# databendlabs/databend

Measured on AMD Instinct MI355X. Metric: rows/s TPC-H Q1 hash-agg, higher is better.
Workload: dtype i64/i128 decimal

## Files before the change

databend_amd/csrc/dev_common.h:

```cpp
#pragma once
#ifndef __HIPCC_RTC__
#include <hip/hip_runtime.h>
#include <stdint.h>
#endif

#ifndef __HIPCC_RTC__
#include "../../include/dbhip.h"
#else
#include "dbhip.h"
#endif

typedef __int128 i128;
typedef unsigned __int128 u128;

#define DBHIP_WAVE 64

#define DBHIP_NULL_HASH_VAL 0xd1cefa08eb382d69ULL

__host__ __device__ __forceinline__ uint64_t agg_hash_u64(uint64_t x) {
  x ^= x >> 32;
  x *= 0xd6e8feb86659fd93ULL;
  x ^= x >> 32;
  x *= 0xd6e8feb86659fd93ULL;
  x ^= x >> 32;
  return x;
}

__host__ __device__ __forceinline__ uint64_t agg_hash_bytes(const uint8_t* p, uint32_t len) {
  const uint64_t M = 0xc6a4a7935bd1e995ULL;
  const uint64_t SEED = 0xe17a1465ULL;
  const int R = 47;
  uint64_t h = SEED ^ ((uint64_t)len * M);
  uint32_t nblocks = len / 8;
  for (uint32_t i = 0; i < nblocks; ++i) {
    uint64_t k = 0;
    for (int b = 0; b < 8; ++b) k |= (uint64_t)p[i * 8 + b] << (8 * b);
    k *= M;
    k ^= k >> R;
    k *= M;
    h ^= k;
    h *= M;
  }
  uint32_t tail = len - nblocks * 8;
  const uint8_t* t = p + nblocks * 8;
  for (uint32_t i = 0; i < tail; ++i) h ^= (uint64_t)t[i] << (8 * (tail - i - 1));
  h ^= h >> R;
  h *= M;
  h ^= h >> R;
  return h;
}

__device__ __forceinline__ uint64_t agg_hash_inline_view(uint32_t len, uint32_t w1, uint32_t w2,
                                                         uint32_t w3) {
  const uint64_t M = 0xc6a4a7935bd1e995ULL;
  const uint64_t SEED = 0xe17a1465ULL;
  const int R = 47;
  uint64_t h = SEED ^ ((uint64_t)len * M);
  uint64_t lo = ((uint64_t)w2 << 32) | w1;
  uint32_t tail_len = len;
  uint64_t tail_src = lo;
  if (len >= 8) {
    uint64_t k = lo;
    k *= M;
    k ^= k >> R;
    k *= M;
    h ^= k;
    h *= M;
    tail_len = len - 8;
    tail_src = w3;
  }
  uint64_t folded = 0;
  for (uint32_t i = 0; i < 7; ++i) {
    if (i < tail_len) folded |= ((tail_src >> (8 * i)) & 0xff) << (8 * (tail_len - i - 1));
  }
  h ^= folded;
  h ^= h >> R;
  h *= M;
  h ^= h >> R;
  return h;
}

__host__ __device__ __forceinline__ uint64_t agg_hash_i256(uint64_t w0, uint64_t w1, uint64_t w2, uint64_t w3) {
  const uint64_t M = 0xc6a4a7935bd1e995ULL;
  const uint64_t SEED = 0xe17a1465ULL;
  const int R = 47;
  uint64_t h = SEED ^ (32ULL * M);
  const uint64_t w[4] = {w0, w1, w2, w3};
#pragma unroll
  for (int i = 0; i < 4; ++i) {
    uint64_t k = w[i];
    k *= M;
    k ^= k >> R;
    k *= M;
    h ^= k;
    h *= M;
  }
  h ^= h >> R;
  h *= M;
  h ^= h >> R;
  return h;
}

__device__ __forceinline__ uint64_t agg_hash_i128(i128 v) {
  const uint64_t M = 0xc6a4a7935bd1e995ULL;
  const uint64_t SEED = 0xe17a1465ULL;
  const int R = 47;
  uint64_t h = SEED ^ (16ULL * M);
  uint64_t w[2] = {(uint64_t)(u128)v, (uint64_t)((u128)v >> 64)};
#pragma unroll
  for (int i = 0; i < 2; ++i) {
    uint64_t k = w[i];
    k *= M;
    k ^= k >> R;
    k *= M;
    h ^= k;
    h *= M;
  }
  h ^= h >> R;
  h *= M;
  h ^= h >> R;
  return h;
}

__host__ __device__ __forceinline__ uint64_t merge_hash(uint64_t a, uint64_t b) {
  return a * DBHIP_NULL_HASH_VAL ^ b;
}

__device__ __forceinline__ bool bit_get(const uint8_t* bm, int64_t i) {
  return (bm[i >> 3] >> (i & 7)) & 1;
}

__device__ __forceinline__ uint64_t wave_sum_u64(uint64_t v) {
#pragma unroll
  for (int off = 32; off >= 1; off >>= 1) v += __shfl_xor(v, off, 64);
  return v;
}

__device__ __forceinline__ u128 wave_sum_u128(u128 v) {
#pragma unroll
  for (int off = 32; off >= 1; off >>= 1) {
    uint64_t lo = __shfl_xor((uint64_t)v, off, 64);
    uint64_t hi = __shfl_xor((uint64_t)(v >> 64), off, 64);
    v += ((u128)hi << 64) | lo;
  }
  return v;
}

__device__ __forceinline__ u128 wave_sum_u192(u128 v, uint64_t* ext) {
  uint64_t e = *ext;
#pragma unroll
  for (int off = 32; off >= 1; off >>= 1) {
    uint64_t lo = __shfl_xor((uint64_t)v, off, 64);
    uint64_t hi = __shfl_xor((uint64_t)(v >> 64), off, 64);
    uint64_t oe = __shfl_xor(e, off, 64);
    u128 o = ((u128)hi << 64) | lo;
    u128 r = v + o;
    e += oe + (r < v ? 1 : 0);
    v = r;
  }
  *ext = e;
  return v;
}

__device__ __forceinline__ int lane_id() { return threadIdx.x & 63; }

struct u256 {
  u128 lo, hi;
};

__host__ __device__ __forceinline__ u256 u256_mul_128(u128 a, u128 b) {
  uint64_t a0 = (uint64_t)a, a1 = (uint64_t)(a >> 64);
  uint64_t b0 = (uint64_t)b, b1 = (uint64_t)(b >> 64);
  u128 p00 = (u128)a0 * b0;
  u128 p01 = (u128)a0 * b1;
  u128 p10 = (u128)a1 * b0;
  u128 p11 = (u128)a1 * b1;
  u128 mid = (p00 >> 64) + (uint64_t)p01 + (uint64_t)p10;
  u256 r;
  r.lo = ((u128)(uint64_t)mid << 64) | (uint64_t)p00;
  r.hi = p11 + (p01 >> 64) + (p10 >> 64) + (mid >> 64);
  return r;
}

__host__ __device__ __forceinline__ u256 u256_add_128(u256 a, u128 b) {
  u256 r;
  r.lo = a.lo + b;
  r.hi = a.hi + (r.lo < a.lo ? 1 : 0);
  return r;
}

__host__ __device__ __forceinline__ bool u256_lt_128(u256 a, u128 b) { return a.hi == 0 && a.lo < b; }

__host__ __device__ __forceinline__ u256 u256_sub_128(u256 a, u128 b) {
  u256 r;
  r.lo = a.lo - b;
  r.hi = a.hi - (a.lo < b ? 1 : 0);
  return r;
}

__host__ __device__ inline uint64_t udiv_2by1(uint64_t u1, uint64_t u0, uint64_t v, uint64_t* rem) {
  const double dv = (double)v;
  const double e = ((double)u1 * 18446744073709551616.0 + (double)u0) / dv;
  uint64_t q = e >= 18446744073709549568.0 ? ~0ULL : (uint64_t)e;
  const u128 n = ((u128)u1 << 64) | u0;
  i128 r = (i128)(n - (u128)q * (u128)v);
  const u128 mag = r < 0 ? (u128)0 - (u128)r : (u128)r;
  const double dm = (double)(uint64_t)(mag >> 64) * 18446744073709551616.0 + (double)(uint64_t)mag;
  const double er = (r < 0 ? -dm : dm) / dv;
  int64_t c = (int64_t)er;
  if ((double)c > er) --c;
  q += (uint64_t)c;
  r -= (i128)c * (i128)(u128)v;
  if (r < 0) { --q; r += (i128)(u128)v; }
  else if (r >= (i128)(u128)v) { ++q; r -= (i128)(u128)v; }
  if (rem) *rem = (uint64_t)r;
  return q;
}

__host__ __device__ inline u128 udiv128_by_64(u128 n, uint64_t d, uint64_t* rem) {
  const uint64_t nh = (uint64_t)(n >> 64), nl = (uint64_t)n;
  uint64_t r = 0;
  const uint64_t qh = nh ? udiv_2by1(0, nh, d, &r) : 0;
  const uint64_t ql = udiv_2by1(r, nl, d, rem);
  return ((u128)qh << 64) | ql;
}

__host__ __device__ inline u256 u256_div_128(u256 a, u128 d, u128* rem) {
  u256 q;
  q.lo = 0;
  q.hi = 0;
  if (a.hi == 0) {
    if ((uint64_t)(d >> 64) == 0) {
      uint64_t r64;
      q.lo = udiv128_by_64(a.lo, (uint64_t)d, &r64);
      if (rem) *rem = r64;
      return q;
    }
    q.lo = a.lo / d;
    if (rem) *rem = a.lo % d;
    return q;
  }
  u128 r = 0;
  for (int i = 255; i >= 0; --i) {
    bool carry = (r >> 127) & 1;
    r <<= 1;
    u128 bit = (i >= 128) ? ((a.hi >> (i - 128)) & 1) : ((a.lo >> i) & 1);
    r |= bit;
    if (carry || r >= d) {
      r -= d;
      if (i >= 128)
        q.hi |= ((u128)1 << (i - 128));
      else
        q.lo |= ((u128)1 << i);
    }
  }
  if (rem) *rem = r;
  return q;
}

static __device__ const uint64_t kDbhipPow10[39][2] = {
  {0x0000000000000001ULL, 0x0000000000000000ULL},
  {0x000000000000000aULL, 0x0000000000000000ULL},
  {0x0000000000000064ULL, 0x0000000000000000ULL},
  {0x00000000000003e8ULL, 0x0000000000000000ULL},
  {0x0000000000002710ULL, 0x0000000000000000ULL},
  {0x00000000000186a0ULL, 0x0000000000000000ULL},
  {0x00000000000f4240ULL, 0x0000000000000000ULL},
  {0x0000000000989680ULL, 0x0000000000000000ULL},
  {0x0000000005f5e100ULL, 0x0000000000000000ULL},
  {0x000000003b9aca00ULL, 0x0000000000000000ULL},
  {0x00000002540be400ULL, 0x0000000000000000ULL},
  {0x000000174876e800ULL, 0x0000000000000000ULL},
  {0x000000e8d4a51000ULL, 0x0000000000000000ULL},
  {0x000009184e72a000ULL, 0x0000000000000000ULL},
  {0x00005af3107a4000ULL, 0x0000000000000000ULL},
  {0x00038d7ea4c68000ULL, 0x0000000000000000ULL},
  {0x002386f26fc10000ULL, 0x0000000000000000ULL},
  {0x016345785d8a0000ULL, 0x0000000000000000ULL},
  {0x0de0b6b3a7640000ULL, 0x0000000000000000ULL},
  {0x8ac7230489e80000ULL, 0x0000000000000000ULL},
  {0x6bc75e2d63100000ULL, 0x0000000000000005ULL},
  {0x35c9adc5dea00000ULL, 0x0000000000000036ULL},
  {0x19e0c9bab2400000ULL, 0x000000000000021eULL},
  {0x02c7e14af6800000ULL, 0x000000000000152dULL},
  {0x1bcecceda1000000ULL, 0x000000000000d3c2ULL},
  {0x161401484a000000ULL, 0x0000000000084595ULL},
  {0xdcc80cd2e4000000ULL, 0x000000000052b7d2ULL},
  {0x9fd0803ce8000000ULL, 0x00000000033b2e3cULL},
  {0x3e25026110000000ULL, 0x00000000204fce5eULL},
  {0x6d7217caa0000000ULL, 0x00000001431e0faeULL},
  {0x4674edea40000000ULL, 0x0000000c9f2c9cd0ULL},
  {0xc0914b2680000000ULL, 0x0000007e37be2022ULL},
  {0x85acef8100000000ULL, 0x000004ee2d6d415bULL},
  {0x38c15b0a00000000ULL, 0x0000314dc6448d93ULL},
  {0x378d8e6400000000ULL, 0x0001ed09bead87c0ULL},
  {0x2b878fe800000000ULL, 0x0013426172c74d82ULL},
  {0xb34b9f1000000000ULL, 0x00c097ce7bc90715ULL},
  {0x00f436a000000000ULL, 0x0785ee10d5da46d9ULL},
  {0x098a224000000000ULL, 0x4b3b4ca85a86c47aULL}};
__host__ __device__ __forceinline__ i128 pow10_i128(int k) {
#if defined(__HIP_DEVICE_COMPILE__)
  k = k < 0 ? 0 : (k > 38 ? 38 : k);
  return (i128)(((u128)kDbhipPow10[k][1] << 64) | kDbhipPow10[k][0]);
#else
  i128 r = 1;
  for (int i = 0; i < k; ++i) r *= 10;
  return r;
#endif
}
```

databend_amd/csrc/dev_decimal.h:

```cpp
#pragma once
#include "dev_common.h"

struct DecOp {
  int op;
  int a_from_scale, a_to_scale, a_to_precision, a_check;
  int b_from_scale, b_to_scale, b_to_precision, b_check;
  int t_is_128;
  int ret_precision, ret_scale;
  int overflow;
  int scale_mul;
  int trivial;
};

__host__ __device__ __forceinline__ i128 wrap_T(i128 v, bool t128) { return t128 ? v : (i128)(int64_t)v; }

__host__ __device__ __forceinline__ i128 max_for_precision(int p) { return pow10_i128(p) - 1; }

__host__ __device__ __forceinline__ bool checked_mul_T(i128 x, i128 f, bool t128, i128* out) {
  if (!t128) {
    i128 r = x * f;
    if (r > (i128)INT64_MAX || r < (i128)INT64_MIN) return false;
    *out = r;
    return true;
  }
  bool neg = (x < 0) != (f < 0);
  u128 ax = x < 0 ? (u128)0 - (u128)x : (u128)x;
  u128 af = f < 0 ? (u128)0 - (u128)f : (u128)f;
  u256 pr = u256_mul_128(ax, af);
  u128 lim = neg ? ((u128)1 << 127) : (((u128)1 << 127) - 1);
  if (pr.hi != 0 || pr.lo > lim) return false;
  *out = neg ? (i128)((u128)0 - pr.lo) : (i128)pr.lo;
  return true;
}

__host__ __device__ __forceinline__ bool convert_operand(i128 x, bool is_decimal, int from_scale, int to_scale,
                                                int to_precision, int check, bool t128, i128* out) {
  if (!is_decimal) {
    if (to_scale == 0) {
      *out = wrap_T(x, t128);
      return true;
    }
    i128 xt = x;
    if (!t128 && (x > (i128)INT64_MAX || x < (i128)INT64_MIN)) return false;
    i128 r;
    if (!checked_mul_T(xt, pow10_i128(to_scale), t128, &r)) return false;
    i128 mx = max_for_precision(to_precision);
    if (r > mx || r < -mx) return false;
    *out = r;
    return true;
  }
  if (!check) {
    *out = wrap_T(x, t128);
    return true;
  }
  i128 r;
  if (!checked_mul_T(wrap_T(x, t128), pow10_i128(to_scale - from_scale), t128, &r)) return false;
  i128 mx = max_for_precision(to_precision);
  if (r > mx || r < -mx) return false;
  *out = r;
  return true;
}

__host__ __device__ __forceinline__ i128 sdiv128(i128 num, i128 d) {
  const bool neg = (num < 0) != (d < 0);
  const u128 un = num < 0 ? (u128)0 - (u128)num : (u128)num;
  const u128 ud = d < 0 ? (u128)0 - (u128)d : (u128)d;
  u128 q;
  if ((uint64_t)(ud >> 64) == 0) q = udiv128_by_64(un, (uint64_t)ud, nullptr);
  else q = un / ud;
  return neg ? (i128)((u128)0 - q) : (i128)q;
}

__device__ bool round_mul_128_overflow(i128 a, i128 b, int shift, i128* out) {
  bool neg = (a < 0) != (b < 0);
  u128 A = a < 0 ? (u128)0 - (u128)a : (u128)a;
  u128 B = b < 0 ? (u128)0 - (u128)b : (u128)b;
  u128 div = (u128)pow10_i128(shift);
  u256 pr = u256_add_128(u256_mul_128(A, B), div / 2);
  u256 q = u256_div_128(pr, div, nullptr);
  u128 lim = neg ? ((u128)1 << 127) : (((u128)1 << 127) - 1);
  if (q.hi != 0 || q.lo > lim) return false;
  *out = neg ? (i128)((u128)0 - q.lo) : (i128)q.lo;
  return true;
}

__device__ i128 round_div_128(i128 a, i128 b, int mul_scale) {
  bool neg = (a < 0) != (b < 0);
  u128 A = a < 0 ? (u128)0 - (u128)a : (u128)a;
  u128 B = b < 0 ? (u128)0 - (u128)b : (u128)b;
  u256 num = u256_add_128(u256_mul_128(A, (u128)pow10_i128(mul_scale)), B / 2);
  u256 q = u256_div_128(num, B, nullptr);
  return neg ? (i128)((u128)0 - q.lo) : (i128)q.lo;
}

__device__ __forceinline__ bool dec_row(const DecOp& p, i128 av, i128 bv, bool a_dec, bool b_dec, bool t128, i128* out) {
  i128 a, b, r = 1;
    bool ok = convert_operand(av, a_dec, p.a_from_scale,
                              p.a_to_scale, p.a_to_precision, p.a_check, t128, &a);
    ok = convert_operand(bv, b_dec, p.b_from_scale,
                         p.b_to_scale, p.b_to_precision, p.b_check, t128, &b) && ok;
    if (ok) {
      switch (p.op) {
        case DBHIP_OP_PLUS:
        case DBHIP_OP_MINUS: {
          i128 t = p.op == DBHIP_OP_PLUS ? (i128)((u128)a + (u128)b) : (i128)((u128)a - (u128)b);
          t = wrap_T(t, t128);
          if (p.overflow) {
            i128 mx = max_for_precision(p.ret_precision);
            if (t < -mx || t > mx) ok = false;
          }
          r = t;
        } break;
        case DBHIP_OP_MULTIPLY: {
          if (p.scale_mul == 0) {
            r = wrap_T((i128)((u128)a * (u128)b), t128);
          } else if (!t128) {
            i128 div = pow10_i128(p.scale_mul);
            if (!p.overflow) {
              int64_t prod = (int64_t)((uint64_t)(int64_t)a * (uint64_t)(int64_t)b);
              int64_t d = (int64_t)div;
              int64_t num = ((a < 0) == (b < 0)) ? (int64_t)((uint64_t)prod + (uint64_t)(d / 2))
                                                 : (int64_t)((uint64_t)prod - (uint64_t)(d / 2));
              r = (i128)(num / d);
            } else {
              i128 num = ((a < 0) == (b < 0)) ? a * b + div / 2 : a * b - div / 2;
              i128 res = sdiv128(num, div);
              i128 mx = max_for_precision(18);
              if (res < -mx || res > mx) ok = false;
              r = res;
            }
          } else {
            if (!p.overflow) {
              i128 div = pow10_i128(p.scale_mul);
              i128 prod = (i128)((u128)a * (u128)b);
              i128 num = ((a < 0) == (b < 0)) ? (i128)((u128)prod + (u128)(div / 2))
                                              : (i128)((u128)prod - (u128)(div / 2));
              r = sdiv128(num, div);
            } else {
              ok = round_mul_128_overflow(a, b, p.scale_mul, &r);
            }
          }
        } break;
        default: {
          if (b == 0) {
            ok = false;
          } else if (!t128) {
            i128 mul = pow10_i128(p.scale_mul);
            i128 am = (i128)((u128)a * (u128)mul);
            i128 num = ((a < 0) == (b < 0)) ? (i128)((u128)am + (u128)(b / 2))
                                            : (i128)((u128)am - (u128)(b / 2));
            r = (i128)(int64_t)sdiv128(num, b);
          } else {
            r = round_div_128(a, b, p.scale_mul);
          }
        } break;
      }
    }
    *out = r;
    return ok;
}


__device__ __forceinline__ bool dec_row_nodiv(const DecOp& p, i128 av, i128 bv, bool a_dec, bool b_dec, bool t128, i128* out) {
  i128 a, b, r = 1;
  bool ok = convert_operand(av, a_dec, p.a_from_scale, p.a_to_scale, p.a_to_precision, p.a_check, t128, &a);
  ok = convert_operand(bv, b_dec, p.b_from_scale, p.b_to_scale, p.b_to_precision, p.b_check, t128, &b) && ok;
  if (ok) {
    if (p.op == DBHIP_OP_MULTIPLY) {
      r = wrap_T((i128)((u128)a * (u128)b), t128);
    } else {
      i128 t = p.op == DBHIP_OP_PLUS ? (i128)((u128)a + (u128)b) : (i128)((u128)a - (u128)b);
      t = wrap_T(t, t128);
      if (p.overflow) {
        const i128 mx = max_for_precision(p.ret_precision);
        if (t < -mx || t > mx) ok = false;
      }
      r = t;
    }
  }
  *out = r;
  return ok;
}
__host__ __device__ inline bool dec_op_needs_division(const DecOp& p) { return p.op == DBHIP_OP_DIVIDE || (p.op == DBHIP_OP_MULTIPLY && p.scale_mul != 0); }

int32_t dbhip_decimal_decode_internal(int op, int a_type, int a_prec, int a_scale, int b_type, int b_prec, int b_scale,
                                      DecOp* out, int* out_type, int* out_precision, int* out_scale);
```

Baseline: 95.18 billion.

## Use precomputed reciprocal division for decimal power-of-ten scaling

Replaces the double-based 128-by-64 division with a Moller-Granlund style reciprocal-multiply 2-by-1 division. Normalized divisors and reciprocals for powers of ten up to 10^19 are precomputed in a device table. Decimal multiply rescaling and the 256-bit overflow path use this table instead of the generic division. Wave-uniform ballot checks skip the high-word division when no lane needs it, at the cost of extra code and a table lookup.

Measured after the change: 95.19 billion (median of 3 runs). Within noise of the previous version (+0.0%).

```diff
diff --git a/databend_amd/csrc/dev_common.h b/databend_amd/csrc/dev_common.h
--- a/databend_amd/csrc/dev_common.h
+++ b/databend_amd/csrc/dev_common.h
@@ -217,25 +217,101 @@
   return q;
 }
 
+struct UdivPre {
+  uint64_t dn, v;
+  uint32_t s;
+};
+
+#if defined(UDIV_WAVE_ANY)
+#elif defined(__HIP_DEVICE_COMPILE__)
+#define UDIV_WAVE_ANY(c) (__builtin_amdgcn_ballot_w64(c) != 0)
+#else
+#define UDIV_WAVE_ANY(c) (c)
+#endif
+
+__host__ __device__ inline UdivPre udiv_pre_make(uint64_t d) {
+  UdivPre p;
+  p.s = (uint32_t)__builtin_clzll(d);
+  p.dn = d << p.s;
+  const uint64_t dn = p.dn;
+  const double x = 18446744073709551616.0 / (double)dn;
+  const double v0 = (x - 1.0) * 18446744073709551616.0 - 16384.0;
+  uint64_t v = (uint64_t)(v0 < 0.0 ? 0.0 : v0);
+  u128 R = ~(u128)0 - (((u128)dn << 64) + (u128)v * (u128)dn);
+  const double dm = (double)(uint32_t)(R >> 64) * 18446744073709551616.0 + (double)(uint64_t)R;
+  uint32_t c = (uint32_t)(dm * x * 5.421010862427522170037e-20);
+  c = c ? c - 1 : 0;
+  v += c;
+  R -= (u128)((uint64_t)c * (dn >> 32)) * 4294967296ULL + (uint64_t)c * (uint64_t)(uint32_t)dn;
+  if (R >= (u128)dn) { ++v; R -= (u128)dn; }
+  if (R >= (u128)dn) { ++v; R -= (u128)dn; }
+  p.v = v;
+  return p;
+}
+
+__host__ __device__ __forceinline__ uint64_t udiv_2by1_pre(uint64_t u1, uint64_t u0, uint64_t dn, uint64_t v, uint64_t* rem) {
+  const u128 q = (u128)v * (u128)u1 + (((u128)u1 << 64) | u0);
+  uint64_t q1 = (uint64_t)(q >> 64) + 1;
+  uint64_t r = u0 - q1 * dn;
+  if (r > (uint64_t)q) { --q1; r += dn; }
+  if (r >= dn) { ++q1; r -= dn; }
+  *rem = r;
+  return q1;
+}
+
+__host__ __device__ inline u128 udiv128_by_64_pre(u128 n, const UdivPre& p, uint64_t* rem) {
+  const uint64_t nh = (uint64_t)(n >> 64), nl = (uint64_t)n;
+  const uint32_t s = p.s;
+  const uint64_t n2 = (nh >> 1) >> (63 - s);
+  const uint64_t n1 = (nh << s) | ((nl >> 1) >> (63 - s));
+  const uint64_t n0 = nl << s;
+  uint64_t qh = 0, r = n1;
+  if (UDIV_WAVE_ANY(n2 != 0 || n1 >= p.dn)) qh = udiv_2by1_pre(n2, n1, p.dn, p.v, &r);
+  const uint64_t ql = udiv_2by1_pre(r, n0, p.dn, p.v, &r);
+  if (rem) *rem = r >> s;
+  return ((u128)qh << 64) | ql;
+}
+
+__host__ __device__ inline void udiv256_by_64_pre(u128 hi, u128 lo, const UdivPre& p, u128* qhi, u128* qlo, uint64_t* rem) {
+  if (!UDIV_WAVE_ANY(hi != 0)) {
+    *qhi = 0;
+    *qlo = udiv128_by_64_pre(lo, p, rem);
+    return;
+  }
+  const uint32_t s = p.s;
+  u128 h = hi, l = lo, qh = 0, ql = 0;
+  uint64_t r = ((uint64_t)(h >> 64) >> 1) >> (63 - s);
+#pragma unroll 1
+  for (int i = 0; i < 4; ++i) {
+    const uint64_t w = ((uint64_t)(h >> 64) << s) | (((uint64_t)h >> 1) >> (63 - s));
+    const uint64_t q = udiv_2by1_pre(r, w, p.dn, p.v, &r);
+    qh = (qh << 64) | (ql >> 64);
+    ql = (ql << 64) | q;
+    h = (h << 64) | (l >> 64);
+    l <<= 64;
+  }
+  *qhi = qh;
+  *qlo = ql;
+  if (rem) *rem = r >> s;
+}
+
 __host__ __device__ inline u128 udiv128_by_64(u128 n, uint64_t d, uint64_t* rem) {
-  const uint64_t nh = (uint64_t)(n >> 64), nl = (uint64_t)n;
-  uint64_t r = 0;
-  const uint64_t qh = nh ? udiv_2by1(0, nh, d, &r) : 0;
-  const uint64_t ql = udiv_2by1(r, nl, d, rem);
-  return ((u128)qh << 64) | ql;
+  const UdivPre p = udiv_pre_make(d);
+  return udiv128_by_64_pre(n, p, rem);
 }
 
 __host__ __device__ inline u256 u256_div_128(u256 a, u128 d, u128* rem) {
   u256 q;
   q.lo = 0;
   q.hi = 0;
+  if ((uint64_t)(d >> 64) == 0) {
+    const UdivPre p = udiv_pre_make((uint64_t)d);
+    uint64_t r64;
+    udiv256_by_64_pre(a.hi, a.lo, p, &q.hi, &q.lo, &r64);
+    if (rem) *rem = r64;
+    return q;
+  }
   if (a.hi == 0) {
-    if ((uint64_t)(d >> 64) == 0) {
-      uint64_t r64;
-      q.lo = udiv128_by_64(a.lo, (uint64_t)d, &r64);
-      if (rem) *rem = r64;
-      return q;
-    }
     q.lo = a.lo / d;
     if (rem) *rem = a.lo % d;
     return q;
@@ -298,6 +374,36 @@
   {0xb34b9f1000000000ULL, 0x00c097ce7bc90715ULL},
   {0x00f436a000000000ULL, 0x0785ee10d5da46d9ULL},
   {0x098a224000000000ULL, 0x4b3b4ca85a86c47aULL}};
+#define UDIV_POW10_PRE_MAX 19
+static __device__ const uint64_t kDbhipPow10Pre[UDIV_POW10_PRE_MAX + 1][3] = {
+  {0x8000000000000000ULL, 0xffffffffffffffffULL, 63ULL},
+  {0xa000000000000000ULL, 0x9999999999999999ULL, 60ULL},
+  {0xc800000000000000ULL, 0x47ae147ae147ae14ULL, 57ULL},
+  {0xfa00000000000000ULL, 0x0624dd2f1a9fbe76ULL, 54ULL},
+  {0x9c40000000000000ULL, 0xa36e2eb1c432ca57ULL, 50ULL},
+  {0xc350000000000000ULL, 0x4f8b588e368f0846ULL, 47ULL},
+  {0xf424000000000000ULL, 0x0c6f7a0b5ed8d36bULL, 44ULL},
+  {0x9896800000000000ULL, 0xad7f29abcaf48578ULL, 40ULL},
+  {0xbebc200000000000ULL, 0x5798ee2308c39df9ULL, 37ULL},
+  {0xee6b280000000000ULL, 0x12e0be826d694b2eULL, 34ULL},
+  {0x9502f90000000000ULL, 0xb7cdfd9d7bdbab7dULL, 30ULL},
+  {0xba43b74000000000ULL, 0x5fd7fe17964955fdULL, 27ULL},
+  {0xe8d4a51000000000ULL, 0x19799812dea11197ULL, 24ULL},
+  {0x9184e72a00000000ULL, 0xc25c268497681c26ULL, 20ULL},
+  {0xb5e620f480000000ULL, 0x6849b86a12b9b01eULL, 17ULL},
+  {0xe35fa931a0000000ULL, 0x203af9ee756159b2ULL, 14ULL},
+  {0x8e1bc9bf04000000ULL, 0xcd2b297d889bc2b6ULL, 10ULL},
+  {0xb1a2bc2ec5000000ULL, 0x70ef54646d496892ULL, 7ULL},
+  {0xde0b6b3a76400000ULL, 0x2725dd1d243aba0eULL, 4ULL},
+  {0x8ac7230489e80000ULL, 0xd83c94fb6d2ac34aULL, 0ULL}};
+__device__ __forceinline__ UdivPre udiv_pre_pow10(int k) {
+  UdivPre p;
+  k = k < 0 ? 0 : k;
+  p.dn = kDbhipPow10Pre[k][0];
+  p.v = kDbhipPow10Pre[k][1];
+  p.s = (uint32_t)kDbhipPow10Pre[k][2];
+  return p;
+}
 __host__ __device__ __forceinline__ i128 pow10_i128(int k) {
 #if defined(__HIP_DEVICE_COMPILE__)
   k = k < 0 ? 0 : (k > 38 ? 38 : k);
diff --git a/databend_amd/csrc/dev_decimal.h b/databend_amd/csrc/dev_decimal.h
--- a/databend_amd/csrc/dev_decimal.h
+++ b/databend_amd/csrc/dev_decimal.h
@@ -71,13 +71,22 @@
   return neg ? (i128)((u128)0 - q) : (i128)q;
 }
 
+__device__ __forceinline__ i128 sdiv128_pow10(i128 num, int k) {
+  if (k > UDIV_POW10_PRE_MAX) return sdiv128(num, pow10_i128(k));
+  const u128 un = num < 0 ? (u128)0 - (u128)num : (u128)num;
+  const u128 q = udiv128_by_64_pre(un, udiv_pre_pow10(k), nullptr);
+  return num < 0 ? (i128)((u128)0 - q) : (i128)q;
+}
+
 __device__ bool round_mul_128_overflow(i128 a, i128 b, int shift, i128* out) {
   bool neg = (a < 0) != (b < 0);
   u128 A = a < 0 ? (u128)0 - (u128)a : (u128)a;
   u128 B = b < 0 ? (u128)0 - (u128)b : (u128)b;
   u128 div = (u128)pow10_i128(shift);
   u256 pr = u256_add_128(u256_mul_128(A, B), div / 2);
-  u256 q = u256_div_128(pr, div, nullptr);
+  u256 q;
+  if (shift <= UDIV_POW10_PRE_MAX) udiv256_by_64_pre(pr.hi, pr.lo, udiv_pre_pow10(shift), &q.hi, &q.lo, nullptr);
+  else q = u256_div_128(pr, div, nullptr);
   u128 lim = neg ? ((u128)1 << 127) : (((u128)1 << 127) - 1);
   if (q.hi != 0 || q.lo > lim) return false;
   *out = neg ? (i128)((u128)0 - q.lo) : (i128)q.lo;
@@ -124,7 +133,7 @@
               r = (i128)(num / d);
             } else {
               i128 num = ((a < 0) == (b < 0)) ? a * b + div / 2 : a * b - div / 2;
-              i128 res = sdiv128(num, div);
+              i128 res = sdiv128_pow10(num, p.scale_mul);
               i128 mx = max_for_precision(18);
               if (res < -mx || res > mx) ok = false;
               r = res;
@@ -135,7 +144,7 @@
               i128 prod = (i128)((u128)a * (u128)b);
               i128 num = ((a < 0) == (b < 0)) ? (i128)((u128)prod + (u128)(div / 2))
                                               : (i128)((u128)prod - (u128)(div / 2));
-              r = sdiv128(num, div);
+              r = sdiv128_pow10(num, p.scale_mul);
             } else {
               ok = round_mul_128_overflow(a, b, p.scale_mul, &r);
             }
```
